# domainxz/top-k-rec

Measured on AMD Instinct MI355X. Metric: BPR training triplets/sec (sampler + plan + step), MovieLens-10M shape, higher is better.
Workload: dtype f32

## Files before the change

### top-k-rec_amd/csrc/topk_refine.hip

```cpp
#include "topk_refine.h"

#include <stdlib.h>

#include <algorithm>
#include <type_traits>

#include "topk_parts.h"

namespace tkr {

#ifdef TKR_R2_PROF
__device__ unsigned long long g_r2_prof[8];
#define R2_MARK(i) { const unsigned long long n_ = __builtin_amdgcn_s_memtime(); r2p[i] += n_ - r2t; r2t = n_; }
#else
#define R2_MARK(i)
#endif

constexpr int kSeg = 32;
constexpr int kF2Batch = 40;

__device__ __forceinline__ uint32_t ord16(uint32_t raw) { return (raw & 0x8000u) ? (~raw & 0xffffu) : (raw | 0x8000u); }
__device__ __forceinline__ uint32_t unord16(uint32_t o) { return (o & 0x8000u) ? (o & 0x7fffu) : (~o & 0xffffu); }

__device__ __forceinline__ uint32_t xor32(uint32_t v, int lane) {
    typedef uint32_t u32x2_ __attribute__((ext_vector_type(2)));
    const u32x2_ r = __builtin_amdgcn_permlane32_swap(v, v, false, false);
    return (lane & 32) ? r.x : r.y;
}

template <int SIZE, int STRIDE>
__device__ __forceinline__ void cmpx32(uint32_t& k, int lane) {
    const uint32_t o = lane_xor<STRIDE>(k);
    const bool upper = (lane & STRIDE) != 0, desc = (lane & SIZE) == 0;
    k = (upper != desc) ? max(k, o) : min(k, o);
}
__device__ __forceinline__ uint32_t wave_sort_desc32(uint32_t k, int lane) {
    cmpx32<2, 1>(k, lane);
    cmpx32<4, 2>(k, lane); cmpx32<4, 1>(k, lane);
    cmpx32<8, 4>(k, lane); cmpx32<8, 2>(k, lane); cmpx32<8, 1>(k, lane);
    cmpx32<16, 8>(k, lane); cmpx32<16, 4>(k, lane); cmpx32<16, 2>(k, lane); cmpx32<16, 1>(k, lane);
    cmpx32<32, 16>(k, lane); cmpx32<32, 8>(k, lane); cmpx32<32, 4>(k, lane); cmpx32<32, 2>(k, lane); cmpx32<32, 1>(k, lane);
    cmpx32<64, 32>(k, lane); cmpx32<64, 16>(k, lane); cmpx32<64, 8>(k, lane); cmpx32<64, 4>(k, lane); cmpx32<64, 2>(k, lane);
    cmpx32<64, 1>(k, lane);
    return k;
}

__device__ __forceinline__ float trim_user2_sort(const uint32_t* ent, int uq, int n0, int n1, int K, int lane, float thr_in, float m2,
                                                 uint32_t& key, int& keep) {
    const int n = n0 + n1;
    const int slot = lane < n0 ? lane : kSeg + (lane - n0);
    key = 0;
    if (lane < n) {
        const uint32_t e = ent[slot * kR2Users + uq];
        key = (ord16(e >> 16) << 16) | (e & 0xffffu);
    }
    int lane_here = lane;
    asm volatile("" : "+v"(lane_here));
    key = wave_sort_desc32(key, lane_here);
    keep = n;
    float refined = thr_in;
    if (n >= K) {
        const uint32_t kb = (uint32_t)__builtin_amdgcn_readlane((int)key, K - 1) >> 16;
        refined = fmaxf(thr_in, unordered_bits(kb << 16) - m2);
        const uint32_t ck = ordered_bits(refined) >> 16;
        keep = __popcll(__ballot(lane < n && (key >> 16) >= ck));
    }
    return refined;
}
__device__ __forceinline__ void trim_user2_deal(uint32_t* ent, int uq, uint32_t key, int keep, int c0, int lane) {
    if (lane < keep) ent[(lane < c0 ? lane : kSeg + (lane - c0)) * kR2Users + uq] = (unord16(key >> 16) << 16) | (key & 0xffffu);
}

__device__ __forceinline__ float trim_all2(uint32_t* ent, int uw, int h, int K, float thr, float m2, int& cnt) {
    const int n_mine = cnt;
    const int lane = 32 * h;
    const int n = n_mine + (int)xor32((uint32_t)n_mine, lane);
    uint32_t xo[16];
    const uint32_t tkey = ordered_bits(thr) >> 16;
    uint32_t unlike = 0;
    uint32_t* seg = ent + (h * kSeg) * kR2Users + uw;
#pragma unroll
    for (int e = 0; e < 16; ++e) {
        uint32_t e0 = seg[(2 * e) * kR2Users], e1 = seg[(2 * e + 1) * kR2Users];
        asm volatile("" : "+v"(e0), "+v"(e1));
        const uint32_t k0 = (2 * e < n_mine) ? ord16(e0 >> 16) : 0u;
        const uint32_t k1 = (2 * e + 1 < n_mine) ? ord16(e1 >> 16) : 0u;
        unlike |= ((2 * e < n_mine) ? (k0 ^ tkey) : 0u) | ((2 * e + 1 < n_mine) ? (k1 ^ tkey) : 0u);
        xo[e] = k0 | (k1 << 16);
    }
    uint32_t mixed = unlike & 0x8000u;
    mixed |= xor32(mixed, lane);
    const int s1 = mixed ? 1 : 0;
    const uint32_t top_bit = mixed ? 0u : (tkey & 0x8000u);
    u16x2 mx = {0, 0};
#pragma unroll
    for (int e = 0; e < 16; ++e) {
        xo[e] = ((xo[e] >> s1) & 0x7fff7fffu) | 0x80008000u;
        const u16x2 o = __builtin_bit_cast(u16x2, xo[e]);
        mx = u16x2{(unsigned short)max(mx.x, o.x), (unsigned short)max(mx.y, o.y)};
    }
    uint32_t hi = (uint32_t)max(mx.x, mx.y) & 0x7fffu;
    hi = max(hi, xor32(hi, lane));
    const uint32_t lo = (tkey >> s1) & 0x7fffu;
    const uint32_t differ = (n >= K) ? (lo ^ hi) : 0u;
    const uint32_t every = wave_or(differ);
    const int top = 31 - __clz((int)(every | 1u));
    uint32_t prefix = hi & ~((2u << top) - 1u);
#pragma unroll 1
    for (int b = top; b >= 0; --b) {
        const uint32_t cand = prefix | (1u << b);
        const uint32_t cand2 = cand | (cand << 16);
        u16x2 acc = {0, 0};
#pragma unroll
        for (int e = 0; e < 16; ++e) acc = count_ge2(xo[e], cand2, acc);
        int c = (int)acc.x + (int)acc.y;
        c += (int)xor32((uint32_t)c, lane);
        if (c >= K) prefix = cand;
    }
    const bool active = n >= K && prefix != 0;
    const uint32_t ob = mixed ? (prefix << 17) : ((top_bit | prefix) << 16);
    const float refined = fmaxf(thr, unordered_bits(ob) - m2);
    prefix = min(prefix, ((ordered_bits(refined) >> 16) >> s1) & 0x7fffu);
    if (!active) return thr;
    uint32_t* wq = seg;
    int kept = 0;
#pragma unroll
    for (int e = 0; e < 32; ++e) {
        const uint32_t k15 = ((e & 1) ? (xo[e >> 1] >> 16) : xo[e >> 1]) & 0x7fffu;
        if (k15 >= prefix) {
            const uint32_t v = seg[e * kR2Users];
            *wq = v;
            wq += kR2Users;
            ++kept;
        }
    }
    cnt = kept;
    return refined;
}

template <bool MASKED, int R>
struct Visit2 {
    static __device__ __forceinline__ void run(const uint64_t (&hr)[16], uint32_t hits, const f32x16& sc, uint32_t& wp, uint32_t himask, int col0) {
        if (hr[R]) {
            asm volatile("" ::: "memory");
            uint64_t m = hr[R];
            if constexpr (MASKED) m = __ballot((hits & (1u << R)) != 0u);
            uint64_t saved;
            uint32_t e;
            asm volatile("s_and_saveexec_b64 %[sv], %[m]\n\t"
                         "v_add_u32 %[e], %[c], %[col0]\n\t"
                         "v_and_or_b32 %[e], %[val], %[hm], %[e]\n\t"
                         "ds_write_b32 %[wp], %[e]\n\t"
                         "v_add_u32 %[wp], 0x200, %[wp]\n\t"
                         "s_mov_b64 exec, %[sv]"
                         : [sv] "=&s"(saved), [e] "=&v"(e), [wp] "+v"(wp)
                         : [m] "s"(m), [c] "n"((R & 3) + 8 * (R >> 2)), [col0] "v"(col0), [val] "v"(sc[R]), [hm] "s"(himask)
                         : "memory", "scc");
        }
        if constexpr (R + 1 < 16) Visit2<MASKED, R + 1>::run(hr, hits, sc, wp, himask, col0);
    }
};
static_assert(kR2Users * 4 == 0x200, "the append's address step is a literal");

template <int R>
struct Visit3 {
    static constexpr int C = (R & 3) + 8 * (R >> 2);
    static __device__ __forceinline__ void run(const uint64_t (&hr)[16], const f32x16& sc, uint32_t mh, uint32_t& wp, uint32_t wlim,
                                               uint32_t& nh, uint32_t himask, int col0) {
        if (hr[R]) {
            asm volatile("" ::: "memory");
            uint64_t saved;
            uint32_t e;
            asm volatile("s_and_saveexec_b64 %[sv], %[m]\n\t"
                         "v_and_b32 %[e], %[bit], %[mh]\n\t"
                         "v_cmp_eq_u32 vcc, 0, %[e]\n\t"
                         "s_and_b64 exec, exec, vcc\n\t"
                         "v_add_u32 %[nh], 1, %[nh]\n\t"
                         "v_cmp_gt_u32 vcc, %[wlim], %[wp]\n\t"
                         "s_and_b64 exec, exec, vcc\n\t"
                         "v_add_u32 %[e], %[c], %[col0]\n\t"
                         "v_and_or_b32 %[e], %[val], %[hm], %[e]\n\t"
                         "ds_write_b32 %[wp], %[e]\n\t"
                         "v_add_u32 %[wp], 0x200, %[wp]\n\t"
                         "s_mov_b64 exec, %[sv]"
                         : [sv] "=&s"(saved), [e] "=&v"(e), [wp] "+v"(wp), [nh] "+v"(nh)
                         : [m] "s"(hr[R]), [bit] "n"(1 << C), [c] "n"(C), [mh] "v"(mh), [wlim] "v"(wlim), [col0] "v"(col0), [val] "v"(sc[R]),
                           [hm] "s"(himask)
                         : "memory", "scc", "vcc");
        }
        if constexpr (R + 1 < 16) Visit3<R + 1>::run(hr, sc, mh, wp, wlim, nh, himask, col0);
    }
};

__device__ __forceinline__ void filter3(uint32_t* ent, const f32x16& sc, uint32_t maskw, int t, int K, float& thr, uint32_t& wp, uint32_t seg0,
                                        float m2, bool& lost, int lane, int wave) {
    const int ul = lane & 31, h = lane >> 5;
    const uint32_t mh = maskw >> (4 * h);
    const uint32_t wlim = seg0 + kSeg * kR2Users * 4, wp_in = wp;
    int col0 = t * 32 + 4 * h;
    asm volatile("" : "+v"(col0));
    const uint32_t himask = 0xffff0000u;
    uint32_t nh = 0;
    {
        uint64_t hr[16], any = 0;
#pragma unroll
        for (int r = 0; r < 16; ++r) { hr[r] = __ballot(sc[r] >= thr); any |= hr[r]; }
        if (!any) return;
#if defined(TKR_R2_ABL) && (TKR_R2_ABL & 2)
        if (any != 12345u) return;
#endif
        Visit3<0>::run(hr, sc, mh, wp, wlim, nh, himask, col0);
    }
    uint64_t ov = __ballot(wp_in + nh * (kR2Users * 4) > wlim);
    if (ov == 0) return;
    uint32_t hits = 0;
#pragma unroll
    for (int r = 0; r < 16; ++r) hits |= (sc[r] >= thr) ? (1u << r) : 0u;
    const uint32_t nm = ~mh;
    hits &= (nm & 0xfu) | ((nm >> 4) & 0xf0u) | ((nm >> 8) & 0xf00u) | ((nm >> 12) & 0xf000u);
    const int written = (int)((wp - wp_in) >> 9);
#pragma unroll
    for (int i = 0; i < 16; ++i)
        if (i < written) hits &= hits - 1u;
    int cnt = (int)((wp - seg0) >> 9);
    int n_mine = __popc(hits);
    const uint64_t hr[16] = {~0ull, ~0ull, ~0ull, ~0ull, ~0ull, ~0ull, ~0ull, ~0ull, ~0ull, ~0ull, ~0ull, ~0ull, ~0ull, ~0ull, ~0ull, ~0ull};
    while (ov) {
        const int u = __builtin_amdgcn_readfirstlane((__ffsll((long long)ov) - 1) & 31);
        const int n0 = __builtin_amdgcn_readlane(cnt, u), n1 = __builtin_amdgcn_readlane(cnt, u + 32);
        uint32_t key;
        int keep;
        const float nt = trim_user2_sort(ent, wave * 32 + u, n0, n1, K, lane, __shfl(thr, u, 64), __shfl(m2, u, 64), key, keep);
        if (ul == u) {
            thr = fmaxf(thr, nt);
            uint32_t still = 0;
#pragma unroll
            for (int r = 0; r < 16; ++r) still |= (sc[r] >= thr) ? (1u << r) : 0u;
            hits &= still;
            n_mine = __popc(hits);
        }
        const int p0 = __builtin_amdgcn_readlane(n_mine, u), p1 = __builtin_amdgcn_readlane(n_mine, u + 32);
        const int lo = max(0, keep - (kSeg - p1)), hi = min(keep, kSeg - p0);
        const bool fits = lo <= hi;
        const int c0 = fits ? min(max((keep + 1) >> 1, lo), hi) : min((keep + 1) >> 1, kSeg);
        trim_user2_deal(ent, wave * 32 + u, key, min(keep, c0 + kSeg), c0, lane);
        if (lane == u) cnt = c0;
        if (lane == u + 32) cnt = min(keep - c0, kSeg);
        if (ul == u && !fits) { lost = true; hits = 0; n_mine = 0; }
        ov &= ~((1ull << u) | (1ull << (u + 32)));
    }
    wp = seg0 + (uint32_t)cnt * (kR2Users * 4);
    Visit2<true, 0>::run(hr, hits, sc, wp, himask, col0);
}

template <int KS>
__global__ __launch_bounds__(256, 3) void score_topk_refine2_kernel(const Refine2Args a) {
    extern __shared__ __attribute__((aligned(16))) unsigned char smem_raw[];
    constexpr int ROWB = KS * 32;
    constexpr int TILEB = 32 * ROWB;
    constexpr int NT_ = 256;
    constexpr int NG = (TILEB / 16 + NT_ - 1) / NT_;
    float* tbias = reinterpret_cast<float*>(smem_raw + 2 * TILEB);
    uint32_t* ent = reinterpret_cast<uint32_t*>(tbias + 64);

    const int tid = threadIdx.x, lane = tid & 63, wave = tid >> 6;
    const int ul = lane & 31, h = lane >> 5;
    const int uw = wave * 32 + ul;
#ifdef TKR_R2_PROF
    unsigned long long r2p[8] = {0, 0, 0, 0, 0, 0, 0, 0}, r2t = __builtin_amdgcn_s_memtime();
#endif
    int4 it = make_int4((int)blockIdx.x, (int)blockIdx.y * a.tiles_per_split, 0, (int)blockIdx.y | ((int)gridDim.y << 16));
    if (a.items) it = a.items[blockIdx.x];
    const int block = it.x, slot = it.w & 0xffff, stride = it.w >> 16;
    const int row = block * kR2Users + uw;
    const bool user_ok = row < a.n_rows;
    const int k = a.k;

    f16x8 hreg[KS];
    float margin, bscale, sv;
    bool sane;
    refine_prologue<KS>(a.U + (size_t)(user_ok ? (a.uidx ? a.uidx[row] : row) : 0) * k, k, user_ok, h, a.extra, hreg, margin, bscale, sv, sane);
    const float m2 = 2.f * margin;
    bool lost = user_ok && !sane;
    const uint32_t seg0 = (uint32_t)(uintptr_t)(ent + (h * kSeg) * kR2Users + uw);
    uint32_t wp = seg0;
    float thr = (a.thr_shared && user_ok) ? unordered_bits(a.thr_shared[row]) : -INFINITY;
    thr = thr * bscale - margin;
    const int n_tiles_all = (a.n_cols + 31) >> 5;
    const int t_begin = it.y;
    const int n_tiles = a.items ? it.z : min(n_tiles_all, t_begin + a.tiles_per_split);

    const int wave_u = __builtin_amdgcn_readfirstlane(wave);
    auto stage_direct = [&](int t, int buf) {
#pragma unroll
        for (int q = 0; q < NG; ++q) {
            const int c0 = q * NT_ + wave_u * 64;
            if ((TILEB / 16) % NT_ == 0 || c0 < TILEB / 16) {
                const int c = min(c0 + lane, TILEB / 16 - 1);
                __builtin_amdgcn_global_load_lds((const __attribute__((address_space(1))) void*)(a.vimg + (size_t)t * TILEB + (size_t)c * 16),
                                                 (__attribute__((address_space(3))) void*)(smem_raw + buf * TILEB + c0 * 16), 16, 0, 0);
            }
        }
    };
    const bool bias_lane = a.bias != nullptr && tid < 32;
    auto bias_of = [&](int t) {
        const int col = t * 32 + tid;
        return (bias_lane && col < a.n_cols) ? a.bias[col] : 0.f;
    };
    if (t_begin < n_tiles) stage_direct(t_begin, t_begin & 1);
    if (bias_lane) tbias[(t_begin & 1) * 32 + tid] = bias_of(t_begin);
    asm volatile("s_waitcnt vmcnt(0)" ::: "memory");
    __syncthreads();

    const uint32_t tail_mask = (a.n_cols & 31) ? (0xffffffffu << (a.n_cols & 31)) : 0u;
    int next_sched = t_begin + 2;
    uint32_t mask_next = (a.mask && user_ok && t_begin < n_tiles) ? a.mask[(size_t)t_begin * a.mask_pitch + row] : 0u;
    R2_MARK(5)
    for (int t = t_begin; t < n_tiles; ++t) {
        const int buf = t & 1;
        uint32_t maskw = mask_next;
        f32x16 acc = {0, 0, 0, 0, 0, 0, 0, 0, 0, 0, 0, 0, 0, 0, 0, 0};
        float bias_next = 0.f;
        if (t + 1 < n_tiles) {
            stage_direct(t + 1, buf ^ 1);
            bias_next = bias_of(t + 1);
        }
        f16x8 afrag[KS];
#pragma unroll
        for (int s = 0; s < KS; ++s)
            afrag[s] = *reinterpret_cast<const f16x8*>(smem_raw + buf * TILEB + ul * ROWB + ((2 * s + h) ^ tile_swizzle<KS>(ul)) * 16);
#pragma unroll
        for (int s = 0; s < KS; ++s) acc = __builtin_amdgcn_mfma_f32_32x32x16_f16(afrag[s], hreg[s], acc, 0, 0, 0);
        __builtin_amdgcn_sched_group_barrier(0x100, KS, 0);
        __builtin_amdgcn_sched_group_barrier(0x008, KS, 0);
        mfma_result_guard_8pass(acc);
        if (a.bias) add_scaled_bias_inplace(acc, tbias + buf * 32, h, bscale);
#ifdef TKR_R2_PROF
        asm volatile("" : "+v"(acc));
        R2_MARK(0)
#endif
        asm volatile("s_waitcnt vmcnt(0)" ::: "memory");
        R2_MARK(1)
        if (bias_lane) tbias[(buf ^ 1) * 32 + tid] = bias_next;
        __syncthreads();
        R2_MARK(2)
        if (a.mask && user_ok && t + 1 < n_tiles) mask_next = a.mask[(size_t)(t + 1) * a.mask_pitch + row];
        if (!user_ok) maskw = 0xffffffffu;
        if (t == n_tiles_all - 1) maskw |= tail_mask;
#if defined(TKR_R2_ABL) && (TKR_R2_ABL & 4)
        if (t == -12345) {
#else
        if (t == next_sched) {
#endif
            int cnt = (int)((wp - seg0) >> 9);
            if (__ballot(cnt + (int)xor32((uint32_t)cnt, lane) > kSeg) != 0) {
                thr = trim_all2(ent, uw, h, a.K, thr, m2, cnt);
                wp = seg0 + (uint32_t)cnt * (kR2Users * 4);
                float bs = bscale;
                int row_here = row;
                asm volatile("" : "+v"(bs), "+v"(row_here));
                thr = share_bound(a.thr_shared, row_here, user_ok && h == 0, thr, margin, bscale,
                                  __uint_as_float((254u - ((__float_as_uint(bs) >> 23) & 0xffu)) << 23));
            }
            next_sched = t + ((t - t_begin + 1) >> 1);
        }
        R2_MARK(3)
#if defined(TKR_R2_ABL) && (TKR_R2_ABL & 1)
        if (acc[0] + acc[5] + acc[10] + acc[15] == 12345.678f) wp += 512;
#else
        filter3(ent, acc, maskw, t, a.K, thr, wp, seg0, m2, lost, lane, wave);
#endif
#ifdef TKR_R2_PROF
        asm volatile("" : "+v"(wp), "+v"(thr));
        R2_MARK(4)
        r2p[7] += 1;
#endif
    }
    int cnt = (int)((wp - seg0) >> 9);
    if (__ballot(lost) != 0 && lane == 0) a.extra[4 + block] = 1u;
    if (__ballot(cnt + (int)xor32((uint32_t)cnt, lane) > kSeg) != 0) {
        thr = trim_all2(ent, uw, h, a.K, thr, m2, cnt);
        thr = share_bound(a.thr_shared, row, user_ok && h == 0, thr, margin, bscale, __uint_as_float((254u - ((__float_as_uint(bscale) >> 23) & 0xffu)) << 23));
    }
    __builtin_amdgcn_wave_barrier();
    const size_t piece = a.pbase ? (size_t)a.pbase[block] + slot : (size_t)block * stride + slot;
    const int n_other = __shfl_xor(cnt, 32, 64);
    if (h == 0 && user_ok) a.dhdr[piece * kR2Users + uw] = make_float2(__int_as_float(cnt | (n_other << 8)), thr);
    for (int u = 0; u < 32; ++u) {
        if (block * kR2Users + wave * 32 + u >= a.n_rows) break;
        const int n0 = __builtin_amdgcn_readlane(cnt, u), n1 = __builtin_amdgcn_readlane(cnt, u + 32);
        if ((lane & 31) < (lane < 32 ? n0 : n1))
            a.dump[(piece * kR2Users + wave * 32 + u) * kR2Slots + lane] = ent[lane * kR2Users + wave * 32 + u];
    }
#ifdef TKR_R2_PROF
    R2_MARK(6)
    if (lane == 0)
        for (int i = 0; i < 8; ++i) atomicAdd(&g_r2_prof[i], r2p[i]);
#endif
}

struct Finish2Args {
    const uint32_t* dump;
    const float2* dhdr;
    int n_rows, S_uniform;
    const int32_t* nslots;
    const int32_t* pbase;
    const uint32_t* flagged;
    const float* U;
    const int32_t* uidx;
    const float* Vt;
    const float* bias;
    int k, K;
    int32_t* out_ids;
    float* out_scores;
};

constexpr int kF2Waves = 2;

template <int KS>
__global__ __launch_bounds__(kF2Waves * 64) void topk_finish2_kernel(const Finish2Args a) {
    constexpr int NSTEP = KS >= 2 ? KS / 2 : 1;
    constexpr int STAGEB = KS >= 2 ? kF2Batch * 128 : 16;
    constexpr int NI = kF2Batch / 8;
    __shared__ __attribute__((aligned(16))) unsigned char s_stage[kF2Waves][2][STAGEB];
    __shared__ uint32_t s_q[kF2Waves][128];
    __shared__ uint64_t s_key[kF2Waves][64];
    __shared__ __attribute__((aligned(16))) float s_u[kF2Waves][128];
    const int lane = threadIdx.x & 63, wave = __builtin_amdgcn_readfirstlane(threadIdx.x >> 6);
    const int n_waves = gridDim.x * kF2Waves;
    const int k = a.k, K = a.K;
    struct Row { int S; size_t p0; bool skip; float2 hme; uint32_t e0, e1, e2, e3; float4 u4; int ul; const float* up; };
    auto fetch = [&](int r) {
        Row w;
        w.skip = true; w.S = 0; w.p0 = 0; w.ul = 0; w.up = a.U; w.hme = make_float2(0.f, -INFINITY); w.u4 = make_float4(0.f, 0.f, 0.f, 0.f);
        w.e0 = w.e1 = w.e2 = w.e3 = 0u;
        if (r >= a.n_rows) return w;
        const int block = r / kR2Users;
        w.ul = r - block * kR2Users;
        if (a.flagged && a.flagged[block]) return w;
        w.skip = false;
        w.S = a.nslots ? a.nslots[block] : a.S_uniform;
        w.p0 = a.pbase ? (size_t)a.pbase[block] : (size_t)block * a.S_uniform;
        if (lane < w.S) w.hme = a.dhdr[(w.p0 + lane) * kR2Users + w.ul];
        w.e0 = a.dump[(w.p0 * kR2Users + w.ul) * kR2Slots + lane];
        w.e1 = a.dump[((w.p0 + min(1, w.S - 1)) * kR2Users + w.ul) * kR2Slots + lane];
        w.e2 = a.dump[((w.p0 + min(2, w.S - 1)) * kR2Users + w.ul) * kR2Slots + lane];
        w.e3 = a.dump[((w.p0 + min(3, w.S - 1)) * kR2Users + w.ul) * kR2Slots + lane];
        const int urow_i = __builtin_amdgcn_readfirstlane(a.uidx ? a.uidx[r] : r);
        w.up = a.U + (size_t)urow_i * k;
        if constexpr (KS >= 2) {
            if (lane < 4 * KS) w.u4 = reinterpret_cast<const float4*>(w.up)[lane];
        }
        return w;
    };
    int r = __builtin_amdgcn_readfirstlane(blockIdx.x * kF2Waves + wave);
    Row nxt = fetch(r);
    for (; r < a.n_rows; r += n_waves) {
    const Row cur = nxt;
    nxt = fetch(r + n_waves);
    if (cur.skip) continue;
    const int S = cur.S, ul = cur.ul;
    const size_t p0 = cur.p0;
    const float2 hme = cur.hme;
    const float* up = cur.up;
    __builtin_amdgcn_wave_barrier();
    if constexpr (KS >= 2) {
        if (lane < 4 * KS) reinterpret_cast<float4*>(s_u[wave])[lane] = cur.u4;
    }
    float B = lane < S ? hme.y : -INFINITY;
    for (int s0 = 64; s0 < S; s0 += 64)
        if (s0 + lane < S) B = fmaxf(B, a.dhdr[(p0 + s0 + lane) * kR2Users + ul].y);
#pragma unroll
    for (int o = 32; o > 0; o >>= 1) B = fmaxf(B, __shfl_xor(B, o, 64));
    const uint32_t ckB = ordered_bits(B) >> 16;
    uint32_t* q = s_q[wave];
    uint64_t* keys = s_key[wave];
    unsigned char* stage = s_stage[wave][0];
    int queued = 0;
    uint64_t best = 0ull;
    bool first = true, counted = false;
    int s = 0;
    auto flush = [&](int m) {
        const bool live = lane < m;
        const int col = live ? (int)q[lane] : 0;
        float sc;
        if constexpr (KS >= 2) {
            const int KH = 8 * KS;
            int colv[NI];
#pragma unroll
            for (int i = 0; i < NI; ++i) colv[i] = (int)q[min(8 * i + (lane >> 3), m - 1)];
            auto issue = [&](int step, int b) {
#pragma unroll
                for (int i = 0; i < NI; ++i) {
                    const int j = 8 * i + (lane >> 3);
                    const int g = (lane & 7) ^ ((j >> 1) & 7);
                    const float* src = a.Vt + (size_t)colv[i] * k + (g < 4 ? 16 * step + 4 * g : KH + 16 * step + 4 * (g - 4));
                    __builtin_amdgcn_global_load_lds((const __attribute__((address_space(1))) void*)src,
                                                     (__attribute__((address_space(3))) void*)(stage + b * STAGEB + i * 1024), 16, 0, 0);
                }
            };
            asm volatile("" ::: "memory");
            issue(0, 0);
            if (NSTEP > 1) issue(1, 1);
            const int cl = min(lane, kF2Batch - 1);
            const int rot = (cl >> 1) & 7;
            float acc = 0.f;
#pragma unroll
            for (int step = 0; step < NSTEP; ++step) {
                if (step + 1 < NSTEP) asm volatile("s_waitcnt vmcnt(%0)" ::"n"(NI) : "memory");
                else asm volatile("s_waitcnt vmcnt(0)" ::: "memory");
                const unsigned char* blk = stage + (step & 1) * STAGEB + cl * 128;
                float4 v[8];
#pragma unroll
                for (int c = 0; c < 8; ++c) v[c] = *reinterpret_cast<const float4*>(blk + ((c ^ rot) * 16));
                const float4* u0 = reinterpret_cast<const float4*>(s_u[wave] + 16 * step);
                const float4* u1 = reinterpret_cast<const float4*>(s_u[wave] + KH + 16 * step);
#pragma unroll
                for (int c = 0; c < 4; ++c)
                    chain_step4(acc, v[c], v[4 + c], u0[c], u1[c]);
                asm volatile("" : "+v"(acc) : : "memory");
                if (step + 2 < NSTEP) issue(step + 2, step & 1);
            }
            sc = chain_finish(acc, a.bias, col);
        } else {
            sc = live ? exact_score(up, a.Vt + (size_t)col * k, k, a.bias, col) : 0.f;
        }
        const uint64_t mine = live ? (((uint64_t)ordered_bits(sc) << 32) | ((uint32_t)col + 1u)) : 0ull;
        keys[lane] = mine;
        __builtin_amdgcn_wave_barrier();
        if (first && m == queued && s >= S) {
            int rank = 0;
            for (int j = 0; j < m; j += 2) {
                const uint64_t k0 = keys[j], k1 = keys[j + 1];
                rank += (k0 > mine) + (k1 > mine);
            }
            if (live && rank < K) {
                a.out_ids[(size_t)r * K + rank] = col;
                if (a.out_scores) a.out_scores[(size_t)r * K + rank] = sc;
            }
            if (lane >= m && lane < K) {
                a.out_ids[(size_t)r * K + lane] = -1;
                if (a.out_scores) a.out_scores[(size_t)r * K + lane] = -INFINITY;
            }
            queued = 0;
            counted = true;
            return;
        }
        const uint64_t key = keys[lane];
        if (first) {
            best = wave_sort_desc(key, lane);
            first = false;
        } else {
#pragma unroll 1
            for (int hx = 0; hx < 2; ++hx) {
                const uint64_t in = (uint64_t)__shfl((unsigned long long)key, (lane & 31) + 32 * hx, 64);
                best = wave_sort_desc(lane < 32 ? best : in, lane);
            }
        }
        if (lane >= 32) best = 0ull;
        __builtin_amdgcn_wave_barrier();
        const uint32_t rest = (lane + m < queued) ? q[lane + m] : 0u;
        const uint32_t rest2 = (lane + 64 + m < queued) ? q[lane + 64 + m] : 0u;
        __builtin_amdgcn_wave_barrier();
        q[lane] = rest;
        q[lane + 64] = rest2;
        queued -= m;
        __builtin_amdgcn_wave_barrier();
    };
    __builtin_amdgcn_wave_barrier();
    while (s < S || queued > 0) {
        while (s < S && queued < kF2Batch) {
            const size_t at = p0 + s;
            const int nn = s < 64 ? __shfl(__float_as_int(hme.x), s, 64) : __float_as_int(a.dhdr[at * kR2Users + ul].x);
            uint32_t e = s == 0 ? cur.e0 : s == 1 ? cur.e1 : s == 2 ? cur.e2 : cur.e3;
            if (s >= 4) e = a.dump[(at * kR2Users + ul) * kR2Slots + lane];
            const int n_seg = lane < 32 ? (nn & 0xff) : ((nn >> 8) & 0xff);
            const bool keep = (lane & 31) < n_seg && ord16(e >> 16) >= ckB;
            const uint64_t m = __ballot(keep);
            if (keep) q[queued + __popcll(m & ((1ull << lane) - 1ull))] = e & 0xffffu;
            queued += __popcll(m);
            __builtin_amdgcn_wave_barrier();
            ++s;
        }
        if (queued > 0) flush(min(queued, kF2Batch));
    }
    if (counted) continue;
    if (lane < K) {
        const bool have = best != 0ull;
        const uint32_t ob = (uint32_t)(best >> 32);
        const uint32_t f = (ob & 0x80000000u) ? (ob & 0x7fffffffu) : ~ob;
        a.out_ids[(size_t)r * K + lane] = have ? (int32_t)((uint32_t)best - 1u) : -1;
        if (a.out_scores) a.out_scores[(size_t)r * K + lane] = have ? __uint_as_float(f) : -INFINITY;
    }
    }
}

#ifdef TKR_R2_PROF
extern "C" int tkr_k4_prof_read(unsigned long long* out8) {
    unsigned long long zero[8] = {0, 0, 0, 0, 0, 0, 0, 0};
    hipError_t e = hipMemcpyFromSymbol(out8, HIP_SYMBOL(g_r2_prof), sizeof(zero));
    if (e == hipSuccess) e = hipMemcpyToSymbol(HIP_SYMBOL(g_r2_prof), zero, sizeof(zero));
    return (int)e;
}
#endif

size_t refine2_dump_bytes(size_t n_pieces) { return n_pieces * kR2Users * (kR2Slots * sizeof(uint32_t) + sizeof(float2)) + 256; }
bool refine2_supports(int n_cols, int k) { return n_cols <= 65535 && k <= 128; }

template <int KS>
static int launch_tile2(const Refine2Args& a, hipStream_t stream) {
    const size_t lds = (size_t)2 * 32 * KS * 32 + 64 * sizeof(float) + (size_t)kR2Slots * kR2Users * sizeof(uint32_t);
    auto kern = score_topk_refine2_kernel<KS>;
    hipError_t e = hipFuncSetAttribute(reinterpret_cast<const void*>(kern), hipFuncAttributeMaxDynamicSharedMemorySize, 64 * 1024);
    if (e != hipSuccess) return (int)e;
    hipLaunchKernelGGL(kern, dim3(a.grid_x, a.grid_y), dim3(256), lds, stream, a);
    return (int)hipGetLastError();
}

int launch_refine2(const Refine2Args& a, hipStream_t stream) {
    if (!refine2_supports(a.n_cols, a.k) || !a.extra || !a.vimg || !a.dump || !a.dhdr) return TKR_EUNSUPPORTED;
    const int KS = a.k <= 16 ? 1 : (a.k <= 32 ? 2 : (a.k <= 64 ? 4 : 8));
    int rc = KS == 1 ? launch_tile2<1>(a, stream) : KS == 2 ? launch_tile2<2>(a, stream) : KS == 4 ? launch_tile2<4>(a, stream) : launch_tile2<8>(a, stream);
    if (rc != TKR_OK) return rc;
    const Finish2Args f = {a.dump, a.dhdr, a.n_rows, a.grid_y, a.items ? a.nslots : nullptr, a.items ? a.pbase : nullptr, a.extra + 4, a.U, a.uidx,
                           a.Vt, a.bias, a.k, a.K, a.out_ids, a.out_scores};
    const bool staged = a.k == 16 * KS && KS >= 2;
    static const int rows_per_cu = getenv("TKR_TOPK_FINISH_ROWS") ? atoi(getenv("TKR_TOPK_FINISH_ROWS")) : 0;
    auto launch_f = [&](auto kern) {
        int blocks = (a.n_rows + kF2Waves - 1) / kF2Waves;
        if (rows_per_cu > 0) blocks = std::min(blocks, 256 * rows_per_cu);
        hipLaunchKernelGGL(kern, dim3(blocks), dim3(kF2Waves * 64), 0, stream, f);
    };
    if (staged && KS == 8) launch_f(topk_finish2_kernel<8>);
    else if (staged && KS == 4) launch_f(topk_finish2_kernel<4>);
    else if (staged && KS == 2) launch_f(topk_finish2_kernel<2>);
    else launch_f(topk_finish2_kernel<0>);
    return (int)hipGetLastError();
}

}
```

Before: 42.53 million.

## Software-pipeline refine2 tile loop: overlap next-tile MFMA with current bias and threshold ballots

Restructures the top-k refine2 tile loop so the MFMA for tile t+1 is issued while tile t's bias add and threshold ballots run interleaved between MFMAs. Staging moves two tiles ahead, and the bias buffer becomes a 4-deep ring. The bias path is also made a template parameter. This targets MFMA latency stalls in the scoring loop, at the cost of more registers (two accumulators) and more LDS. However, the metric here is BPR training throughput, and this top-k kernel likely is not on that path.

```diff
diff --git a/top-k-rec_amd/csrc/topk_refine.hip b/top-k-rec_amd/csrc/topk_refine.hip
--- a/top-k-rec_amd/csrc/topk_refine.hip
+++ b/top-k-rec_amd/csrc/topk_refine.hip
@@ -17,6 +17,7 @@
 #endif
 
 constexpr int kSeg = 32;
+constexpr int kBiasRing = 4;
 constexpr int kF2Batch = 40;
 
 __device__ __forceinline__ uint32_t ord16(uint32_t raw) { return (raw & 0x8000u) ? (~raw & 0xffffu) : (raw | 0x8000u); }
@@ -43,6 +44,21 @@
     cmpx32<64, 32>(k, lane); cmpx32<64, 16>(k, lane); cmpx32<64, 8>(k, lane); cmpx32<64, 4>(k, lane); cmpx32<64, 2>(k, lane);
     cmpx32<64, 1>(k, lane);
     return k;
+}
+
+typedef float f32x4 __attribute__((ext_vector_type(4)));
+__device__ __forceinline__ void read_bias_ring(f32x4 (&bq)[4], const float* tbias, int h) {
+    const uint32_t at = (uint32_t)(uintptr_t)(tbias + 4 * h);
+    asm volatile("ds_read_b128 %0, %4\n\t"
+                 "ds_read_b128 %1, %4 offset:32\n\t"
+                 "ds_read_b128 %2, %4 offset:64\n\t"
+                 "ds_read_b128 %3, %4 offset:96\n\t"
+                 "s_waitcnt lgkmcnt(0)"
+                 : "=&v"(bq[0]), "=&v"(bq[1]), "=&v"(bq[2]), "=&v"(bq[3]) : "v"(at) : "memory");
+}
+__device__ __forceinline__ float fma_bias(float x, float b, float bscale) {
+    asm("v_fma_f32 %0, %1, %2, %0" : "+v"(x) : "v"(b), "v"(bscale));
+    return x;
 }
 
 __device__ __forceinline__ float trim_user2_sort(const uint32_t* ent, int uq, int n0, int n1, int K, int lane, float thr_in, float m2,
@@ -192,8 +208,8 @@
     }
 };
 
-__device__ __forceinline__ void filter3(uint32_t* ent, const f32x16& sc, uint32_t maskw, int t, int K, float& thr, uint32_t& wp, uint32_t seg0,
-                                        float m2, bool& lost, int lane, int wave) {
+__device__ __forceinline__ void filter3(uint32_t* ent, const f32x16& sc, const uint64_t (&hr)[16], uint64_t any, uint32_t maskw, int t, int K,
+                                        float& thr, uint32_t& wp, uint32_t seg0, float m2, bool& lost, int lane, int wave) {
     const int ul = lane & 31, h = lane >> 5;
     const uint32_t mh = maskw >> (4 * h);
     const uint32_t wlim = seg0 + kSeg * kR2Users * 4, wp_in = wp;
@@ -202,9 +218,6 @@
     const uint32_t himask = 0xffff0000u;
     uint32_t nh = 0;
     {
-        uint64_t hr[16], any = 0;
-#pragma unroll
-        for (int r = 0; r < 16; ++r) { hr[r] = __ballot(sc[r] >= thr); any |= hr[r]; }
         if (!any) return;
 #if defined(TKR_R2_ABL) && (TKR_R2_ABL & 2)
         if (any != 12345u) return;
@@ -224,7 +237,7 @@
         if (i < written) hits &= hits - 1u;
     int cnt = (int)((wp - seg0) >> 9);
     int n_mine = __popc(hits);
-    const uint64_t hr[16] = {~0ull, ~0ull, ~0ull, ~0ull, ~0ull, ~0ull, ~0ull, ~0ull, ~0ull, ~0ull, ~0ull, ~0ull, ~0ull, ~0ull, ~0ull, ~0ull};
+    const uint64_t all[16] = {~0ull, ~0ull, ~0ull, ~0ull, ~0ull, ~0ull, ~0ull, ~0ull, ~0ull, ~0ull, ~0ull, ~0ull, ~0ull, ~0ull, ~0ull, ~0ull};
     while (ov) {
         const int u = __builtin_amdgcn_readfirstlane((__ffsll((long long)ov) - 1) & 31);
         const int n0 = __builtin_amdgcn_readlane(cnt, u), n1 = __builtin_amdgcn_readlane(cnt, u + 32);
@@ -250,10 +263,10 @@
         ov &= ~((1ull << u) | (1ull << (u + 32)));
     }
     wp = seg0 + (uint32_t)cnt * (kR2Users * 4);
-    Visit2<true, 0>::run(hr, hits, sc, wp, himask, col0);
-}
-
-template <int KS>
+    Visit2<true, 0>::run(all, hits, sc, wp, himask, col0);
+}
+
+template <int KS, bool BIAS>
 __global__ __launch_bounds__(256, 3) void score_topk_refine2_kernel(const Refine2Args a) {
     extern __shared__ __attribute__((aligned(16))) unsigned char smem_raw[];
     constexpr int ROWB = KS * 32;
@@ -261,7 +274,7 @@
     constexpr int NT_ = 256;
     constexpr int NG = (TILEB / 16 + NT_ - 1) / NT_;
     float* tbias = reinterpret_cast<float*>(smem_raw + 2 * TILEB);
-    uint32_t* ent = reinterpret_cast<uint32_t*>(tbias + 64);
+    uint32_t* ent = reinterpret_cast<uint32_t*>(tbias + kBiasRing * 32);
 
     const int tid = threadIdx.x, lane = tid & 63, wave = tid >> 6;
     const int ul = lane & 31, h = lane >> 5;
@@ -296,8 +309,9 @@
         for (int q = 0; q < NG; ++q) {
             const int c0 = q * NT_ + wave_u * 64;
             if ((TILEB / 16) % NT_ == 0 || c0 < TILEB / 16) {
-                const int c = min(c0 + lane, TILEB / 16 - 1);
-                __builtin_amdgcn_global_load_lds((const __attribute__((address_space(1))) void*)(a.vimg + (size_t)t * TILEB + (size_t)c * 16),
+                uint32_t c16 = (uint32_t)min(c0 + lane, TILEB / 16 - 1) * 16u;
+                asm volatile("" : "+v"(c16));
+                __builtin_amdgcn_global_load_lds((const __attribute__((address_space(1))) void*)(a.vimg + (size_t)t * TILEB + c16),
                                                  (__attribute__((address_space(3))) void*)(smem_raw + buf * TILEB + c0 * 16), 16, 0, 0);
             }
         }
@@ -307,44 +321,53 @@
         const int col = t * 32 + tid;
         return (bias_lane && col < a.n_cols) ? a.bias[col] : 0.f;
     };
-    if (t_begin < n_tiles) stage_direct(t_begin, t_begin & 1);
-    if (bias_lane) tbias[(t_begin & 1) * 32 + tid] = bias_of(t_begin);
-    asm volatile("s_waitcnt vmcnt(0)" ::: "memory");
-    __syncthreads();
-
+    const uint32_t row4 = (uint32_t)row * 4u;
+    auto mask_of = [&](int t) {
+        uint32_t r4 = row4;
+        asm volatile("" : "+v"(r4));
+        return *reinterpret_cast<const uint32_t*>(reinterpret_cast<const char*>(a.mask + (size_t)t * a.mask_pitch) + r4);
+    };
+    auto read_frags = [&](int t, f16x8 (&afrag)[KS]) {
+#pragma unroll
+        for (int s = 0; s < KS; ++s)
+            afrag[s] = *reinterpret_cast<const f16x8*>(smem_raw + (t & 1) * TILEB + ul * ROWB + ((2 * s + h) ^ tile_swizzle<KS>(ul)) * 16);
+    };
     const uint32_t tail_mask = (a.n_cols & 31) ? (0xffffffffu << (a.n_cols & 31)) : 0u;
     int next_sched = t_begin + 2;
-    uint32_t mask_next = (a.mask && user_ok && t_begin < n_tiles) ? a.mask[(size_t)t_begin * a.mask_pitch + row] : 0u;
+    uint32_t mask_next = (a.mask && user_ok && t_begin < n_tiles) ? mask_of(t_begin) : 0u;
+    f32x16 accA, accB;
+    {
+        if (t_begin < n_tiles) stage_direct(t_begin, t_begin & 1);
+        if (bias_lane) tbias[(t_begin & (kBiasRing - 1)) * 32 + tid] = bias_of(t_begin);
+        asm volatile("s_waitcnt vmcnt(0)" ::: "memory");
+        __syncthreads();
+        float bias_next = 0.f;
+        if (t_begin + 1 < n_tiles) {
+            stage_direct(t_begin + 1, (t_begin + 1) & 1);
+            bias_next = bias_of(t_begin + 1);
+        }
+        accA = f32x16{0, 0, 0, 0, 0, 0, 0, 0, 0, 0, 0, 0, 0, 0, 0, 0};
+        if (t_begin < n_tiles) {
+            f16x8 afrag[KS];
+            read_frags(t_begin, afrag);
+#pragma unroll
+            for (int s = 0; s < KS; ++s) accA = __builtin_amdgcn_mfma_f32_32x32x16_f16(afrag[s], hreg[s], accA, 0, 0, 0);
+            __builtin_amdgcn_sched_group_barrier(0x100, KS, 0);
+            __builtin_amdgcn_sched_group_barrier(0x008, KS, 0);
+        }
+        asm volatile("s_waitcnt vmcnt(0)" ::: "memory");
+        if (bias_lane) tbias[((t_begin + 1) & (kBiasRing - 1)) * 32 + tid] = bias_next;
+        __syncthreads();
+    }
     R2_MARK(5)
-    for (int t = t_begin; t < n_tiles; ++t) {
-        const int buf = t & 1;
+    auto step = [&](int t, f32x16& cur, f32x16& nxt) {
         uint32_t maskw = mask_next;
-        f32x16 acc = {0, 0, 0, 0, 0, 0, 0, 0, 0, 0, 0, 0, 0, 0, 0, 0};
         float bias_next = 0.f;
-        if (t + 1 < n_tiles) {
-            stage_direct(t + 1, buf ^ 1);
-            bias_next = bias_of(t + 1);
-        }
-        f16x8 afrag[KS];
-#pragma unroll
-        for (int s = 0; s < KS; ++s)
-            afrag[s] = *reinterpret_cast<const f16x8*>(smem_raw + buf * TILEB + ul * ROWB + ((2 * s + h) ^ tile_swizzle<KS>(ul)) * 16);
-#pragma unroll
-        for (int s = 0; s < KS; ++s) acc = __builtin_amdgcn_mfma_f32_32x32x16_f16(afrag[s], hreg[s], acc, 0, 0, 0);
-        __builtin_amdgcn_sched_group_barrier(0x100, KS, 0);
-        __builtin_amdgcn_sched_group_barrier(0x008, KS, 0);
-        mfma_result_guard_8pass(acc);
-        if (a.bias) add_scaled_bias_inplace(acc, tbias + buf * 32, h, bscale);
-#ifdef TKR_R2_PROF
-        asm volatile("" : "+v"(acc));
-        R2_MARK(0)
-#endif
-        asm volatile("s_waitcnt vmcnt(0)" ::: "memory");
-        R2_MARK(1)
-        if (bias_lane) tbias[(buf ^ 1) * 32 + tid] = bias_next;
-        __syncthreads();
-        R2_MARK(2)
-        if (a.mask && user_ok && t + 1 < n_tiles) mask_next = a.mask[(size_t)(t + 1) * a.mask_pitch + row];
+        if (t + 2 < n_tiles) {
+            stage_direct(t + 2, t & 1);
+            bias_next = bias_of(t + 2);
+        }
+        if (a.mask && user_ok && t + 1 < n_tiles) mask_next = mask_of(t + 1);
         if (!user_ok) maskw = 0xffffffffu;
         if (t == n_tiles_all - 1) maskw |= tail_mask;
 #if defined(TKR_R2_ABL) && (TKR_R2_ABL & 4)
@@ -357,24 +380,62 @@
                 thr = trim_all2(ent, uw, h, a.K, thr, m2, cnt);
                 wp = seg0 + (uint32_t)cnt * (kR2Users * 4);
                 float bs = bscale;
-                int row_here = row;
-                asm volatile("" : "+v"(bs), "+v"(row_here));
+                uint32_t r4 = row4;
+                asm volatile("" : "+v"(bs), "+v"(r4));
+                const int row_here = (int)(r4 >> 2);
                 thr = share_bound(a.thr_shared, row_here, user_ok && h == 0, thr, margin, bscale,
                                   __uint_as_float((254u - ((__float_as_uint(bs) >> 23) & 0xffu)) << 23));
             }
             next_sched = t + ((t - t_begin + 1) >> 1);
         }
         R2_MARK(3)
+        f16x8 afrag[KS];
+        read_frags(t + 1, afrag);
+        __builtin_amdgcn_sched_barrier(0);
+        mfma_result_guard_8pass(cur);
+        f32x4 bq[4];
+        if constexpr (BIAS) read_bias_ring(bq, tbias + (t & (kBiasRing - 1)) * 32, h);
+        uint64_t hr[16], any = 0;
+        nxt = f32x16{0, 0, 0, 0, 0, 0, 0, 0, 0, 0, 0, 0, 0, 0, 0, 0};
+        constexpr int GAPS = KS > 1 ? KS - 1 : 1;
+#pragma unroll
+        for (int s = 0; s < KS; ++s) {
+            nxt = __builtin_amdgcn_mfma_f32_32x32x16_f16(afrag[s], hreg[s], nxt, 0, 0, 0);
+            __builtin_amdgcn_sched_barrier(0);
+            if (s < GAPS) {
+#pragma unroll
+                for (int r = 16 * s / GAPS; r < 16 * (s + 1) / GAPS; ++r) {
+                    if constexpr (BIAS) cur[r] = fma_bias(cur[r], bq[r >> 2][r & 3], bscale);
+                    hr[r] = __ballot(cur[r] >= thr);
+                    any |= hr[r];
+                }
+                __builtin_amdgcn_sched_barrier(0);
+            }
+        }
+        R2_MARK(0)
 #if defined(TKR_R2_ABL) && (TKR_R2_ABL & 1)
-        if (acc[0] + acc[5] + acc[10] + acc[15] == 12345.678f) wp += 512;
+        if (cur[0] + cur[5] + cur[10] + cur[15] == 12345.678f + (float)(any & 1)) wp += 512;
 #else
-        filter3(ent, acc, maskw, t, a.K, thr, wp, seg0, m2, lost, lane, wave);
+        filter3(ent, cur, hr, any, maskw, t, a.K, thr, wp, seg0, m2, lost, lane, wave);
 #endif
 #ifdef TKR_R2_PROF
         asm volatile("" : "+v"(wp), "+v"(thr));
         R2_MARK(4)
         r2p[7] += 1;
 #endif
+        asm volatile("s_waitcnt vmcnt(0)" ::: "memory");
+        R2_MARK(1)
+        if (bias_lane) tbias[((t + 2) & (kBiasRing - 1)) * 32 + tid] = bias_next;
+        __syncthreads();
+        R2_MARK(2)
+    };
+    {
+        int t = t_begin;
+        for (; t + 1 < n_tiles; t += 2) {
+            step(t, accA, accB);
+            step(t + 1, accB, accA);
+        }
+        if (t < n_tiles) step(t, accA, accB);
     }
     int cnt = (int)((wp - seg0) >> 9);
     if (__ballot(lost) != 0 && lane == 0) a.extra[4 + block] = 1u;
@@ -609,8 +670,8 @@
 
 template <int KS>
 static int launch_tile2(const Refine2Args& a, hipStream_t stream) {
-    const size_t lds = (size_t)2 * 32 * KS * 32 + 64 * sizeof(float) + (size_t)kR2Slots * kR2Users * sizeof(uint32_t);
-    auto kern = score_topk_refine2_kernel<KS>;
+    const size_t lds = (size_t)2 * 32 * KS * 32 + kBiasRing * 32 * sizeof(float) + (size_t)kR2Slots * kR2Users * sizeof(uint32_t);
+    auto kern = a.bias ? score_topk_refine2_kernel<KS, true> : score_topk_refine2_kernel<KS, false>;
     hipError_t e = hipFuncSetAttribute(reinterpret_cast<const void*>(kern), hipFuncAttributeMaxDynamicSharedMemorySize, 64 * 1024);
     if (e != hipSuccess) return (int)e;
     hipLaunchKernelGGL(kern, dim3(a.grid_x, a.grid_y), dim3(256), lds, stream, a);
```

After: 41.04 million. 0.965x the previous value.
